# glacierbliss/iceberg_tracking_code

Hardware: AMD Instinct MI355X
Metric: frame_pairs_per_sec (higher is better)
Workload: dtype u8/int32/f32

## Files before the change

### iceberg_tracking_code_amd/build.py

```python
import os
import shutil
import subprocess
import sys
from concurrent.futures import ThreadPoolExecutor

HERE = os.path.dirname(os.path.abspath(__file__))
CSRC = os.path.join(HERE, "csrc")
OBJ = os.path.join(CSRC, "obj")
LIB = os.path.join(HERE, "libicelk.so")
SOURCES = ["icelk_abi.hip", "k_image.hip", "k_pyramid.hip", "k_lk.hip", "k_lk_fast.hip", "k_lk_multi.hip", "k_corners.hip", "k_corners_fast.hip", "k_sort.hip", "k_tail.hip", "k_tracks.hip", "k_utm.hip", "k_mask.hip", "k_grid.hip", "k_cube.hip"]
HEADERS = [os.path.join(CSRC, "icelk_internal.h"), os.path.join(CSRC, "lk_common.h"), os.path.join(CSRC, "lk_fast_tiles.h"), os.path.join(CSRC, "np_sums.h"), os.path.join(HERE, "..", "include", "icelk.h")]
ARCH = "gfx950"
FLAGS = ["--offload-arch=" + ARCH, "-O3", "-fPIC", "-std=c++17", "-ffp-contract=off", "-fno-fast-math",
         "-Wall", "-Wno-unused-result", "-Wno-unused-value"]


def _hipcc():
    exe = shutil.which("hipcc") or "/opt/rocm/bin/hipcc"
    if not os.path.exists(exe):
        raise RuntimeError("hipcc not found: libicelk.so cannot be built (ROCm toolchain required)")
    return exe


def _stale(target, deps):
    if not os.path.exists(target):
        return True
    t = os.path.getmtime(target)
    return any(os.path.getmtime(d) > t for d in deps)


def _compile(src, force):
    obj = os.path.join(OBJ, os.path.splitext(src)[0] + ".o")
    path = os.path.join(CSRC, src)
    if force or _stale(obj, [path] + HEADERS):
        cmd = [_hipcc()] + FLAGS + ["-c", path, "-o", obj]
        subprocess.check_call(cmd)
    return obj


def build(force=False, verbose=False):
    os.makedirs(OBJ, exist_ok=True)
    with ThreadPoolExecutor(max_workers=min(6, len(SOURCES))) as ex:
        objs = list(ex.map(lambda s: _compile(s, force), SOURCES))
    if force or _stale(LIB, objs):
        cmd = [_hipcc(), "--offload-arch=" + ARCH, "-shared", "-fPIC", "-o", LIB] + objs
        subprocess.check_call(cmd)
        if verbose:
            print("built", LIB)
    return LIB


if __name__ == "__main__":
    build(force="--force" in sys.argv, verbose=True)
```

### iceberg_tracking_code_amd/csrc/k_lk_fast.hip

```cpp
#include "lk_fast_tiles.h"

namespace icelk {

namespace {

using namespace lk;
using namespace lkf;

__device__ __forceinline__ float sum_to_float(long long t)
{
    const int hi = (int)(t >> 16), lo = (int)(t & 0xffff);
    return __fadd_rn(__fmul_rn((float)hi, 65536.f), (float)lo);
}

__device__ __forceinline__ int floor_uni(float x)
{
    int i = (int)floorf(x);
    asm volatile("" : "+v"(i));
    return uni(i);
}
__device__ __forceinline__ int floor_uni(float x, float& fx)
{
    fx = floorf(x);
    int i = (int)fx;
    asm volatile("" : "+v"(i));
    return uni(i);
}

template <int WW, int WH>
struct TmplIO {
    using C = Cfg<WW, WH>;
    static constexpr int HP = (C::S + 1) / 2;
    static constexpr int NI = C::TPL * C::S;
    static constexpr bool PACKED = ((NI + 1) / 2 + C::TPL * 2 * HP + 1 + 3) / 4 < (NI + C::TPL * 2 * HP + 1 + 3) / 4;
    static constexpr int NIP = PACKED ? (NI + 1) / 2 : NI;
    static constexpr int NDW = NIP + C::TPL * 2 * HP;
    static constexpr int NQ = (NDW + 1 + 3) / 4;
    static constexpr int LEVEL = NQ * 64;
    static constexpr int WAVES = C::TPL == 1 ? 5 : 3;
    static constexpr bool FITS = (C::LDS_DW * 4 + NQ * 1024) * 4 * WAVES <= 160 * 1024;
    static constexpr int LDS_Q = FITS ? NQ * 64 : 1;
};

template <int WW, int WH>
__device__ __forceinline__ void tmpl_store(const Template<WW, WH, 1>& T, float A11, float A12, float A22,
                                           uint4* __restrict__ dst, int lane)
{
    using IO = TmplIO<WW, WH>;
    using C = Cfg<WW, WH>;
    uint32_t d[IO::NQ * 4];
#pragma unroll
    for (int i = 0; i < IO::NQ * 4; i++) d[i] = 0u;
    d[IO::NDW] = __float_as_uint(lane == 0 ? A11 : (lane == 1 ? A12 : A22));
    constexpr int kSeed = 1 << (W_BITS - 6), kShift = W_BITS - 5;
    if constexpr (IO::PACKED) {
#pragma unroll
        for (int p = 0; p < IO::NIP; p++) {
            const uint32_t lo = (uint32_t)(kSeed - T.Ineg[0][(2 * p) / C::S][(2 * p) % C::S]) >> kShift;
            uint32_t hi = 0u;
            if (2 * p + 1 < IO::NI) hi = (uint32_t)(kSeed - T.Ineg[0][(2 * p + 1) / C::S][(2 * p + 1) % C::S]) << (16 - kShift);
            d[p] = lo | hi;
        }
    } else {
#pragma unroll
        for (int n = 0; n < IO::NI; n++) d[n] = (uint32_t)T.Ineg[0][n / C::S][n % C::S];
    }
#pragma unroll
    for (int k = 0; k < C::TPL; k++) {
#pragma unroll
        for (int q = 0; q < IO::HP; q++) {
            d[IO::NIP + k * 2 * IO::HP + q] = T.Ixp[0][k][q];
            d[IO::NIP + k * 2 * IO::HP + IO::HP + q] = T.Iyp[0][k][q];
        }
    }
    typedef uint32_t u4v __attribute__((ext_vector_type(4)));
#pragma unroll
    for (int q = 0; q < IO::NQ; q++) {
        const u4v v = {d[4 * q], d[4 * q + 1], d[4 * q + 2], d[4 * q + 3]};
        __builtin_nontemporal_store(v, reinterpret_cast<u4v*>(dst + q * 64 + lane));
    }
}

template <int WW, int WH>
__device__ __forceinline__ void tmpl_unpack(Template<WW, WH, 1>& T, float& A11, float& A12, float& A22,
                                            const uint4 (&v)[TmplIO<WW, WH>::NQ])
{
    using IO = TmplIO<WW, WH>;
    using C = Cfg<WW, WH>;
    uint32_t d[IO::NQ * 4];
#pragma unroll
    for (int q = 0; q < IO::NQ; q++) { d[4 * q] = v[q].x; d[4 * q + 1] = v[q].y; d[4 * q + 2] = v[q].z; d[4 * q + 3] = v[q].w; }
    A11 = __uint_as_float((uint32_t)__builtin_amdgcn_readlane((int)d[IO::NDW], 0));
    A12 = __uint_as_float((uint32_t)__builtin_amdgcn_readlane((int)d[IO::NDW], 1));
    A22 = __uint_as_float((uint32_t)__builtin_amdgcn_readlane((int)d[IO::NDW], 2));
    constexpr int kSeed = 1 << (W_BITS - 6), kShift = W_BITS - 5;
#pragma unroll
    for (int n = 0; n < IO::NI; n++) {
        if constexpr (IO::PACKED) {
            const uint32_t w = d[n / 2];
            const uint32_t sh = (n & 1) ? ((w >> (16 - kShift)) & ~((1u << kShift) - 1u)) : ((w & 0xffffu) << kShift);
            T.Ineg[0][n / C::S][n % C::S] = kSeed - (int)sh;
        } else {
            T.Ineg[0][n / C::S][n % C::S] = (int)d[n];
        }
    }
#pragma unroll
    for (int k = 0; k < C::TPL; k++) {
#pragma unroll
        for (int q = 0; q < IO::HP; q++) {
            T.Ixp[0][k][q] = d[IO::NIP + k * 2 * IO::HP + q];
            T.Iyp[0][k][q] = d[IO::NIP + k * 2 * IO::HP + IO::HP + q];
        }
    }
}

template <int WW, int WH, int WHOLE>
__device__ __forceinline__ void chain_sums_t(const float* fsum, int planes, bool pairwise, float (&out)[3], int lane)
{
    constexpr int NPX = WW * WH;
    constexpr int NI = WHOLE / 4, NT = WW - WHOLE, MAXN = NI > NT ? NI : NT, INFL = Cfg<WW, WH>::TPL > 1 ? 16 : 32,
                  RB = INFL / MAXN > 0 ? INFL / MAXN : 1;
    __syncthreads();
    float acc = 0.f;
    const int p = lane / 5, c = lane - 5 * p;
    const bool busy = lane < 5 * planes;
    const int x0 = c < 4 ? c : WHOLE, stride = c < 4 ? 4 : 1, count = busy ? (c < 4 ? NI : NT) : 0;
    const float* src = fsum + (busy ? p : 0) * NPX + x0;
#pragma unroll 1
    for (int y0 = 0; y0 < WH; y0 += RB) {
        float v[RB][MAXN];
#pragma unroll
        for (int r = 0; r < RB; r++)
#pragma unroll
            for (int i = 0; i < MAXN; i++) {
                const bool ok = i < count && y0 + r < WH;
                v[r][i] = ok ? src[(y0 + r) * WW + i * stride] : 0.f;
            }
#pragma unroll
        for (int r = 0; r < RB; r++)
#pragma unroll
            for (int i = 0; i < MAXN; i++) acc = __fadd_rn(acc, v[r][i]);
    }
#pragma unroll
    for (int q = 0; q < 3; q++) {
        if (q >= planes) break;
        const float q0 = __shfl(acc, 5 * q), q1 = __shfl(acc, 5 * q + 1), q2 = __shfl(acc, 5 * q + 2), q3 = __shfl(acc, 5 * q + 3);
        const float t = __shfl(acc, 5 * q + 4);
        out[q] = pairwise ? __fadd_rn(t, __fadd_rn(__fadd_rn(q0, q2), __fadd_rn(q1, q3)))
                          : __fadd_rn(t, __fadd_rn(__fadd_rn(__fadd_rn(q0, q1), q2), q3));
    }
    __syncthreads();
}

template <int WW, int WH>
__device__ __forceinline__ void chain_sums(const float* fsum, int planes, int whole, bool pairwise, float (&out)[3], int lane)
{
    if (whole == (WW & ~3)) chain_sums_t<WW, WH, (WW & ~3)>(fsum, planes, pairwise, out, lane);
    else chain_sums_t<WW, WH, (WW & ~7)>(fsum, planes, pairwise, out, lane);
}

template <int WW, int WH>
__device__ __forceinline__ TrackResult track_point_fast(const Pyramid& PI, const Pyramid& PJ, float p0x, float p0y,
                                                        const LKParams& P, uint32_t* ldsI, uint32_t* ldsJ, int lane,
                                                        bool want_err, uint4* __restrict__ tio, int tmode, uint4* tlds,
                                                        float* fsum = nullptr)
{
    using C = Cfg<WW, WH>;
    using IO = TmplIO<WW, WH>;
    const bool reuse = IO::FITS && tmode == 1;
    int in_lds = -1;
    auto fetch = [&](int level) {
        const unsigned long long sb = reinterpret_cast<unsigned long long>(tio + level * IO::LEVEL);
        const uint4* src = reinterpret_cast<const uint4*>(((unsigned long long)(unsigned)uni((int)(sb >> 32)) << 32) |
                                                          (unsigned)uni((int)sb)) + lane;
        static_for<IO::NQ>([&](auto qq) {
            constexpr int q = qq, grp = q / 4, in = q % 4;
            __builtin_amdgcn_global_load_lds((const __attribute__((address_space(1))) void*)(src + grp * 256),
                                             (__attribute__((address_space(3))) void*)(tlds + grp * 256), 16, in * 1024, 2 );
        });
        in_lds = uni(level);
    };
    if (reuse) fetch(P.top_level);
    constexpr int S = C::S;
    constexpr int R = kMargin;
    const float half_x = (WW - 1) * 0.5f, half_y = (WH - 1) * 0.5f;
    const float FLT_SCALE = 1.f / (1 << 20);
    constexpr bool kSmall = C::TPL * S <= 8;

    int trow[C::TPL], tcol[C::TPL], tlen[C::TPL], joff[C::TPL];
    uint32_t psel[C::TPL][(S + 1) / 2];
#pragma unroll
    for (int k = 0; k < C::TPL; k++) {
        const int t = lane + 64 * k;
        const bool used = t < C::NTASK;
        const int row = used ? t / C::NSEG : 0;
        trow[k] = row;
        tcol[k] = used ? (t - row * C::NSEG) * S : 0;
        tlen[k] = used ? (WW - tcol[k] < S ? WW - tcol[k] : S) : 0;
        joff[k] = row * C::JPD * 4 + tcol[k];
#pragma unroll
        for (int q = 0; q < (S + 1) / 2; q++)
            psel[k][q] = pair_sel(q, tlen[k]);
    }

    constexpr bool kPackSeg = C::TPL >= 3;
    uint32_t segp[C::TPL];
#pragma unroll
    for (int k = 0; k < C::TPL; k++) segp[k] = (uint32_t)trow[k] | ((uint32_t)tcol[k] << 8) | ((uint32_t)tlen[k] << 16);
    auto seg_rows_cols = [&](int (&row)[C::TPL], int (&col)[C::TPL], int (&len)[C::TPL]) {
#pragma unroll
        for (int k = 0; k < C::TPL; k++) {
            uint32_t v = segp[k];
            asm volatile("" : "+v"(v));
            row[k] = (int)(v & 255u);
            col[k] = (int)((v >> 8) & 255u);
            len[k] = (int)(v >> 16);
        }
    };

    TrackResult Rz;
    Rz.status = 1;
    Rz.err = 0.f;
    Rz.iters = 0;
    float sx = 0.f, sy = 0.f;
    Template<WW, WH, 1> T;

    for (int level = P.top_level, scale_bits = __float_as_int(inv_pow2(P.top_level)); level >= 0;
         level--, scale_bits += 1 << 23) {
        const Level LI = PI.lv[level];
        const Level LJ = PJ.lv[level];
        const float scale = __int_as_float(scale_bits);
        float px = p0x * scale, py = p0y * scale;
        if (level == P.top_level) { sx = px; sy = py; }
        else { sx = sx * 2.f; sy = sy * 2.f; }
        px -= half_x; py -= half_y;
        float fpx, fpy;
        const int ipx = floor_uni(px, fpx), ipy = floor_uni(py, fpy);
        if (!origin_ok<WW, WH>(LI, ipx, ipy)) {
            if (level == 0) { Rz.status = 0; Rz.err = 0.f; }
            continue;
        }
        uint32_t wi0, wi1;
        packed_weights<false>(px - fpx, py - fpy, wi0, wi1);

        float nx = sx - half_x, ny = sy - half_y;
        int jx0 = kUnstaged, jy0 = kUnstaged;
        const int ix0 = ipx - 1, iy0 = ipy - 1;
        const bool i_inside = tile_inside(LI, ix0, iy0, C::ITW, C::ITH);
        {
            const int inx = floor_uni(nx), iny = floor_uni(ny);
            const bool j_ok = origin_ok<WW, WH>(LJ, inx, iny);
            const int tjx = inx - R, tjy = iny - R;
            const bool j_inside = j_ok && tile_inside(LJ, tjx, tjy, C::JTW, C::JTH);
            __syncthreads();
            TileRegs<C::IPD, C::ITH> ti;
            TileRegs<C::JPD, C::JTH> tj;
            if (!reuse) {
                if (i_inside) tile_issue(ti, LI, ix0, iy0, lane);
                else tile_issue_reflect(ti, LI, ix0, iy0, lane);
            }
            if (j_inside) tile_issue(tj, LJ, tjx, tjy, lane);
            else if (j_ok) tile_issue_reflect(tj, LJ, tjx, tjy, lane);
            if (!reuse) tile_commit(ti, ldsI, lane);
            if (j_ok) tile_commit(tj, ldsJ, lane);
            if (j_ok) { jx0 = tjx; jy0 = tjy; }
            __syncthreads();
        }

        float A11, A12, A22;
        if (reuse) {
            if (in_lds != level) fetch(level);
            __builtin_amdgcn_s_waitcnt(0x0F70);
            uint4 tq[IO::NQ];
#pragma unroll
            for (int q = 0; q < IO::NQ; q++) tq[q] = tlds[q * 64 + lane];
            tmpl_unpack<WW, WH>(T, A11, A12, A22, tq);
            __builtin_amdgcn_s_waitcnt(0xC07F);
            if (level > 0) fetch(level - 1);
        } else {
            int a11, a12, a22;
            if constexpr (kPackSeg) {
                int row_l[C::TPL], col_l[C::TPL], len_l[C::TPL];
                uint32_t psel_l[C::TPL][(S + 1) / 2];
                seg_rows_cols(row_l, col_l, len_l);
#pragma unroll
                for (int k = 0; k < C::TPL; k++)
#pragma unroll
                    for (int q = 0; q < (S + 1) / 2; q++)
                        psel_l[k][q] = pair_sel(q, len_l[k]);
                template_pixels<WW, WH, 1, 0>(T, ldsI, (uint32_t)uni((int)wi0), (uint32_t)uni((int)wi1),
                                              ix0 & 3, i_inside, ipx, ipy, LI.w, LI.h, row_l, col_l, psel_l, a11, a12, a22, fsum, len_l);
            } else
            template_pixels<WW, WH, 1, 0>(T, ldsI, (uint32_t)uni((int)wi0), (uint32_t)uni((int)wi1),
                                          ix0 & 3, i_inside, ipx, ipy, LI.w, LI.h, trow, tcol, psel, a11, a12, a22, fsum, tlen);
            long long s11, s12, s22;
            if constexpr (kSmall) wave_sum_mat_i64(a11, a12, a22, s11, s12, s22);
            else wave_sum3_i64<1>(a11, a12, a22, s11, s12, s22);
            A11 = sum_to_float(s11) * FLT_SCALE;
            A12 = sum_to_float(s12) * FLT_SCALE;
            A22 = sum_to_float(s22) * FLT_SCALE;
            if (fsum) {
                float o[3];
                chain_sums<WW, WH>(fsum, 3, P.sum_mode == 1 ? (WW & ~3) : (WW & ~7), P.sum_mode == 2, o, lane);
                A11 = __fmul_rn(o[0], FLT_SCALE); A12 = __fmul_rn(o[1], FLT_SCALE); A22 = __fmul_rn(o[2], FLT_SCALE);
            }
        }
        if (IO::FITS && tmode == 2) tmpl_store<WW, WH>(T, A11, A12, A22, tio + level * IO::LEVEL, lane);
        float D = __fsub_rn(__fmul_rn(A11, A22), __fmul_rn(A12, A12));
        const float dif = __fsub_rn(A11, A22);
        const float rad = __fadd_rn(__fmul_rn(dif, dif), __fmul_rn(__fmul_rn(4.f, A12), A12));
        const float tr = __fadd_rn(A22, A11);
        const float approx = (tr - __builtin_amdgcn_sqrtf(rad)) * (1.f / (float)(2 * WW * WH));
        const bool clear_pass = __builtin_amdgcn_ballot_w64(approx > P.min_eig_thr + tr * 2e-6f) != 0 &&
                                !(P.flags & ICELK_FLAG_MIN_EIGENVALS);
        if (!clear_pass) {
            const float minEig = __fdiv_rn(__fsub_rn(tr, sqrtf(rad)), (float)(2 * WW * WH));
            if (P.flags & ICELK_FLAG_MIN_EIGENVALS) Rz.err = minEig;
            if (minEig < P.min_eig_thr) {
                if (level == 0) Rz.status = 0;
                continue;
            }
        }
        if (D < 1.1920928955078125e-07f) {
            if (level == 0) Rz.status = 0;
            continue;
        }
        D = __fdiv_rn(1.f, D);

        float pdx = __builtin_nanf(""), pdy = __builtin_nanf("");
        for (int j = 0; j < P.max_count; j++) {
            float fnx, fny;
            const int inx = floor_uni(nx, fnx), iny = floor_uni(ny, fny);
            if (!origin_ok<WW, WH>(LJ, inx, iny)) {
                if (level == 0) Rz.status = 0;
                break;
            }
            if (!tile_covers(jx0, jy0, inx, iny)) {
                jx0 = inx - R; jy0 = iny - R;
                __syncthreads();
                TileRegs<C::JPD, C::JTH> tj;
                Level LR = LJ;
                asm volatile("" : "+s"(LR.pitch));
                if (tile_inside(LR, jx0, jy0, C::JTW, C::JTH)) tile_issue(tj, LR, jx0, jy0, lane);
                else tile_issue_reflect(tj, LR, jx0, jy0, lane);
                tile_commit(tj, ldsJ, lane);
                __syncthreads();
            }
            Rz.iters++;
            uint32_t wj0, wj1;
            packed_weights<true>(nx - fnx, ny - fny, wj0, wj1);
            const int jb = uni((iny - jy0) * (C::JPD * 4) + (jx0 & 3) + (inx - jx0));
            int b1, b2;
            if constexpr (kPackSeg) {
                int row_l[C::TPL], col_l[C::TPL], len_l[C::TPL], joff_l[C::TPL];
                seg_rows_cols(row_l, col_l, len_l);
#pragma unroll
                for (int k = 0; k < C::TPL; k++) joff_l[k] = row_l[k] * (C::JPD * 4) + col_l[k];
                residual_pixels<WW, WH, 1, 0, false>(T, ldsJ, jb, (uint32_t)uni((int)wj0),
                                                     (uint32_t)uni((int)wj1), joff_l, len_l, b1, b2, fsum, row_l, col_l);
            } else
            residual_pixels<WW, WH, 1, 0, false>(T, ldsJ, jb, (uint32_t)uni((int)wj0),
                                                 (uint32_t)uni((int)wj1), joff, tlen, b1, b2, fsum, trow, tcol);
            long long t1, t2;
            wave_sum2_i64<kSmall ? 8 : 1>(b1, b2, t1, t2);
            float fb1 = sum_to_float(t1) * FLT_SCALE;
            float fb2 = sum_to_float(t2) * FLT_SCALE;
            if (fsum) {
                float o[3];
                chain_sums<WW, WH>(fsum, 2, WW & ~7, true, o, lane);
                fb1 = __fmul_rn(o[0], FLT_SCALE); fb2 = __fmul_rn(o[1], FLT_SCALE);
            }
            const float dx = __fmul_rn(__fsub_rn(__fmul_rn(A12, fb2), __fmul_rn(A22, fb1)), D);
            const float dy = __fmul_rn(__fsub_rn(__fmul_rn(A12, fb1), __fmul_rn(A11, fb2)), D);
            nx = __fadd_rn(nx, dx); ny = __fadd_rn(ny, dy);
            sx = __fadd_rn(nx, half_x); sy = __fadd_rn(ny, half_y);
            const float q = __fadd_rn(__fmul_rn(dx, dx), __fmul_rn(dy, dy));
            bool conv = q < P.eps2_lo;
            if (__builtin_amdgcn_ballot_w64(!conv && !(q > P.eps2_hi)) != 0) {
                asm volatile("" ::: "memory");
                conv = __dadd_rn(__dmul_rn((double)dx, (double)dx), __dmul_rn((double)dy, (double)dy)) <= P.eps2;
            }
            if (conv) break;
            if (fabsf(__fadd_rn(dx, pdx)) <= 0.01f && fabsf(__fadd_rn(dy, pdy)) <= 0.01f) {
                sx = __fsub_rn(sx, __fmul_rn(dx, 0.5f));
                sy = __fsub_rn(sy, __fmul_rn(dy, 0.5f));
                break;
            }
            pdx = dx; pdy = dy;
        }

        if (Rz.status && level == 0 && !(P.flags & ICELK_FLAG_MIN_EIGENVALS)) {
            const float qx = sx - half_x, qy = sy - half_y;
            const int iqx = floor_uni(qx), iqy = floor_uni(qy);
            if (!origin_ok<WW, WH>(LJ, iqx, iqy)) {
                Rz.status = 0;
                continue;
            }
            if (!want_err) continue;
            if (!tile_covers(jx0, jy0, iqx, iqy)) {
                jx0 = iqx - R; jy0 = iqy - R;
                __syncthreads();
                TileRegs<C::JPD, C::JTH> tj;
                if (tile_inside(LJ, jx0, jy0, C::JTW, C::JTH)) tile_issue(tj, LJ, jx0, jy0, lane);
                else tile_issue_reflect(tj, LJ, jx0, jy0, lane);
                tile_commit(tj, ldsJ, lane);
                __syncthreads();
            }
            uint32_t we0, we1;
            packed_weights<true>(qx - (float)iqx, qy - (float)iqy, we0, we1);
            const int jb = uni((iqy - jy0) * (C::JPD * 4) + (jx0 & 3) + (iqx - jx0));
            int es, unused;
            if constexpr (kPackSeg) {
                int row_l[C::TPL], col_l[C::TPL], len_l[C::TPL], joff_l[C::TPL];
                seg_rows_cols(row_l, col_l, len_l);
#pragma unroll
                for (int k = 0; k < C::TPL; k++) joff_l[k] = row_l[k] * (C::JPD * 4) + col_l[k];
                residual_pixels<WW, WH, 1, 0, true>(T, ldsJ, jb, (uint32_t)uni((int)we0),
                                                    (uint32_t)uni((int)we1), joff_l, len_l, es, unused);
            } else
            residual_pixels<WW, WH, 1, 0, true>(T, ldsJ, jb, (uint32_t)uni((int)we0),
                                                (uint32_t)uni((int)we1), joff, tlen, es, unused);
            const float errval = sum_to_float(sum_pick<kSmall, 8>(es));
            Rz.err = __fdiv_rn(__fmul_rn(errval, 1.f), (float)(32 * WW * WH));
        }
    }
    Rz.x = sx;
    Rz.y = sy;
    return Rz;
}

struct LKJobs {
    LKJob job[2];
    int g0, g1;
};

template <int WW, int WH, bool FB, bool SM = false>
__device__ __forceinline__ void lk_fast_body(const LKJobs& JJ, const LKParams& P)
{
    using C = Cfg<WW, WH>;
    constexpr int kTileQ = (C::LDS_DW + 3) / 4;
    __shared__ uint4 lds_q[kTileQ + (SM ? 1 : TmplIO<WW, WH>::LDS_Q)];
    uint4* const tlds = lds_q + kTileQ;
    __shared__ float fs_[SM ? 3 * WW * WH : 1];
    float* const fsum = SM ? fs_ : nullptr;
    int which = 0, b = blockIdx.x;
    if (JJ.g1 > 0) {
        const int G = b >> 3, m = (JJ.g0 < JJ.g1 ? JJ.g0 : JJ.g1) >> 3;
        const int mb = m & ~31;
        int Gj;
        if (G < 2 * mb) {
            which = (G >> 5) & 1;
            Gj = ((G >> 6) << 5) | (G & 31);
        } else if (G < 2 * m) {
            const int r = G - 2 * mb;
            which = r & 1;
            Gj = mb + (r >> 1);
        } else {
            which = JJ.g0 < JJ.g1 ? 1 : 0;
            Gj = G - m;
        }
        b = (Gj << 3) | (b & 7);
    }
    const LKJob& J = JJ.job[which];
    const LKBuffers& B = J.B;
    const int f = __builtin_amdgcn_readfirstlane(launch_slot(B, b, B.n_dev ? *B.n_dev : J.n));
    if (f < 0) return;
    if (B.seg_alive && !B.seg_alive[f]) return;
    const int lane = threadIdx.x;
    uint32_t* ldsJ = reinterpret_cast<uint32_t*>(lds_q);
    uint32_t* ldsI = ldsJ + C::J_DW;
    const float p0x = B.p_in[2 * f], p0y = B.p_in[2 * f + 1];
    if (lane == 0) stamp(B, 0);
    using IO = TmplIO<WW, WH>;
    const size_t t_off = (size_t)f * ((size_t)B.tmpl_levels * IO::LEVEL);
    const TrackResult r1 = track_point_fast<WW, WH>(J.I, J.J, p0x, p0y, P, ldsI, ldsJ, lane, B.err_fwd != nullptr,
                                                    const_cast<uint4*>(static_cast<const uint4*>(B.tmpl_in)) + t_off,
                                                    !SM && B.tmpl_in ? 1 : 0, tlds, fsum);
    if (lane == 0) {
        if (B.p_fwd) { B.p_fwd[2 * f] = r1.x; B.p_fwd[2 * f + 1] = r1.y; }
        if (B.st_fwd) B.st_fwd[f] = (uint8_t)r1.status;
        if (B.err_fwd) B.err_fwd[f] = r1.err;
        if (B.iters && !FB) B.iters[f] = (uint32_t)r1.iters;
    }
    if (FB) {
        const TrackResult r2 = track_point_fast<WW, WH>(J.J, J.I, r1.x, r1.y, P, ldsI, ldsJ, lane, B.err_bwd != nullptr,
                                                        static_cast<uint4*>(B.tmpl_out) + t_off, !SM && B.tmpl_out ? 2 : 0, tlds,
                                                        fsum);
        if (lane == 0) {
            if (B.p_bwd) { B.p_bwd[2 * f] = r2.x; B.p_bwd[2 * f + 1] = r2.y; }
            if (B.st_bwd) B.st_bwd[f] = (uint8_t)r2.status;
            if (B.err_bwd) B.err_bwd[f] = r2.err;
            if (B.iters) B.iters[f] = (uint32_t)r1.iters | ((uint32_t)r2.iters << 16);
            const float d = fb_distance(p0x, p0y, r2.x, r2.y, P.dist_form);
            if (B.dist) B.dist[f] = d;
            if (B.valid) B.valid[f] = d < P.fb_thr ? 1 : 0;
            if (B.seg_alive) seg_append(B, f, r1.x, r1.y, d, d < P.fb_thr);
        }
    }
    if (lane == 0) stamp(B, 1);
}

template <int WW, int WH, bool FB>
__global__ __launch_bounds__(64, 3) void k_lk_fast(LKJobs JJ, LKParams P)
{
    lk_fast_body<WW, WH, FB>(JJ, P);
}

template <int WW, int WH, bool FB>
__global__ __launch_bounds__(64, 4) __attribute__((amdgpu_num_vgpr(44))) void k_lk_fast88(LKJobs JJ, LKParams P)
{
    lk_fast_body<WW, WH, FB>(JJ, P);
}

template <int WW, int WH, bool FB>
__global__ __launch_bounds__(64, 2) void k_lk_fast_sums(LKJobs JJ, LKParams P)
{
    lk_fast_body<WW, WH, FB, true>(JJ, P);
}

int grid_of(const LKBuffers& B, int n) { return B.order ? (n + 15) & ~7 : (n + 7) & ~7; }

template <int WW, int WH>
void launch_fast(hipStream_t s, const LKJob& a, const LKJob* b, const LKParams& P, bool fb)
{
    LKJobs JJ;
    JJ.job[0] = a;
    JJ.job[1] = b ? *b : a;
    JJ.g0 = grid_of(a.B, a.n);
    JJ.g1 = b ? grid_of(b->B, b->n) : 0;
    const int grid = JJ.g0 + JJ.g1;
    if (P.sum_mode) {
        if (fb) hipLaunchKernelGGL((k_lk_fast_sums<WW, WH, true>), dim3(grid), dim3(64), 0, s, JJ, P);
        else hipLaunchKernelGGL((k_lk_fast_sums<WW, WH, false>), dim3(grid), dim3(64), 0, s, JJ, P);
        return;
    }
    if constexpr (Cfg<WW, WH>::TPL == 1) {
        if (fb) hipLaunchKernelGGL((k_lk_fast88<WW, WH, true>), dim3(grid), dim3(64), 0, s, JJ, P);
        else hipLaunchKernelGGL((k_lk_fast88<WW, WH, false>), dim3(grid), dim3(64), 0, s, JJ, P);
    } else {
        if (fb) hipLaunchKernelGGL((k_lk_fast<WW, WH, true>), dim3(grid), dim3(64), 0, s, JJ, P);
        else hipLaunchKernelGGL((k_lk_fast<WW, WH, false>), dim3(grid), dim3(64), 0, s, JJ, P);
    }
}

bool dispatch_fast(hipStream_t s, const LKJob& a, const LKJob* b, const LKParams& P, bool fb)
{
    if (P.flags & ICELK_FLAG_INITIAL_FLOW) return false;
    if (P.win_w == 21 && P.win_h == 21) launch_fast<21, 21>(s, a, b, P, fb);
    else if (P.win_w == 31 && P.win_h == 31) launch_fast<31, 31>(s, a, b, P, fb);
    else if (P.win_w == 35 && P.win_h == 35) launch_fast<35, 35>(s, a, b, P, fb);
    else if (P.win_w == 15 && P.win_h == 15) launch_fast<15, 15>(s, a, b, P, fb);
    else return false;
    return true;
}

}

int lk_template_quads(int win_w, int win_h)
{
    if (win_w == 21 && win_h == 21) return TmplIO<21, 21>::FITS ? TmplIO<21, 21>::NQ : 0;
    if (win_w == 31 && win_h == 31) return TmplIO<31, 31>::FITS ? TmplIO<31, 31>::NQ : 0;
    if (win_w == 35 && win_h == 35) return TmplIO<35, 35>::FITS ? TmplIO<35, 35>::NQ : 0;
    if (win_w == 15 && win_h == 15) return TmplIO<15, 15>::FITS ? TmplIO<15, 15>::NQ : 0;
    return 0;
}

bool lk_fast_eligible(const LKParams& P)
{
    if (P.flags & (ICELK_FLAG_INITIAL_FLOW | ICELK_FLAG_GENERIC_KERNEL | ICELK_FLAG_MULTI_PER_WAVE)) return false;
    return P.sum_mode == 0 && lk_template_quads(P.win_w, P.win_h) > 0;
}

bool launch_lk_fast(hipStream_t s, const Pyramid& I, const Pyramid& J, const LKBuffers& B, int n, const LKParams& P,
                    bool fb)
{
    LKJob a;
    a.I = I;
    a.J = J;
    a.B = B;
    a.n = n;
    return dispatch_fast(s, a, nullptr, P, fb);
}

bool launch_lk_pair(hipStream_t s, const LKJob& a, const LKJob& b, const LKParams& P)
{
    if (P.flags & (ICELK_FLAG_GENERIC_KERNEL | ICELK_FLAG_MULTI_PER_WAVE)) return false;
    if (a.n <= 0 || b.n <= 0) return false;
    return dispatch_fast(s, a, &b, P, true);
}

}
```

### iceberg_tracking_code_amd/csrc/lk_common.h

```cpp
#pragma once
#include "icelk_internal.h"

namespace icelk {
namespace lk {

constexpr int W_BITS = 14;

__device__ __forceinline__ int reflect101(int p, int n)
{
    if (n == 1) return 0;
    while (p < 0 || p >= n) p = p < 0 ? -p : 2 * n - 2 - p;
    return p;
}

__device__ __forceinline__ int descale(int v, int n) { return (v + (1 << (n - 1))) >> n; }

struct Weights {
    int w00, w01, w10, w11;
};

__device__ __forceinline__ Weights bilinear_weights(float a, float b)
{
    Weights w;
    w.w00 = (int)rintf((1.f - a) * (1.f - b) * (float)(1 << W_BITS));
    w.w01 = (int)rintf(a * (1.f - b) * (float)(1 << W_BITS));
    w.w10 = (int)rintf((1.f - a) * b * (float)(1 << W_BITS));
    w.w11 = (1 << W_BITS) - w.w00 - w.w01 - w.w10;
    return w;
}

struct TrackResult {
    float x, y;
    float err;
    int status;
    int iters;
};

__device__ __forceinline__ int wave_sum_i32(int v)
{
    v += __builtin_amdgcn_update_dpp(0, v, 0x111, 0xf, 0xf, true);
    v += __builtin_amdgcn_update_dpp(0, v, 0x112, 0xf, 0xf, true);
    v += __builtin_amdgcn_update_dpp(0, v, 0x114, 0xf, 0xf, true);
    v += __builtin_amdgcn_update_dpp(0, v, 0x118, 0xf, 0xf, true);
    v += __builtin_amdgcn_update_dpp(0, v, 0x142, 0xa, 0xf, true);
    v += __builtin_amdgcn_update_dpp(0, v, 0x143, 0xc, 0xf, true);
    return __builtin_amdgcn_readlane(v, 63);
}

template <int G>
__device__ __forceinline__ long long wave_sum_grouped(int v)
{
    static_assert(G == 8 || G == 16, "group size");
    v += __builtin_amdgcn_update_dpp(0, v, 0x111, 0xf, 0xf, true);
    v += __builtin_amdgcn_update_dpp(0, v, 0x112, 0xf, 0xf, true);
    v += __builtin_amdgcn_update_dpp(0, v, 0x114, 0xf, 0xf, true);
    if (G == 16) v += __builtin_amdgcn_update_dpp(0, v, 0x118, 0xf, 0xf, true);
    long long t = 0;
#pragma unroll
    for (int g = 0; g < 64 / G; g++) t += (long long)__builtin_amdgcn_readlane(v, g * G + G - 1);
    return t;
}

#define ICELK_DPP64_PAIR(LO, HI, CTRL) \
    "v_add_co_u32_dpp " LO ", vcc, " LO ", " LO " " CTRL "\n\tv_addc_co_u32_dpp " HI ", vcc, " HI ", " HI ", vcc " CTRL "\n\t"
#define ICELK_DPP_SHR8 "row_shr:8 row_mask:0xf bank_mask:0xf bound_ctrl:0"
#define ICELK_DPP_BC15 "row_bcast:15 row_mask:0xa bank_mask:0xf"
#define ICELK_DPP_BC31 "row_bcast:31 row_mask:0xc bank_mask:0xf"

template <int G>
__device__ __forceinline__ int dpp_low_steps(int v)
{
    static_assert(G == 1 || G == 8 || G == 16, "group size");
    if (G >= 8) {
        v += __builtin_amdgcn_update_dpp(0, v, 0x111, 0xf, 0xf, true);
        v += __builtin_amdgcn_update_dpp(0, v, 0x112, 0xf, 0xf, true);
        v += __builtin_amdgcn_update_dpp(0, v, 0x114, 0xf, 0xf, true);
    }
    if (G == 16) v += __builtin_amdgcn_update_dpp(0, v, 0x118, 0xf, 0xf, true);
    return v;
}

__device__ __forceinline__ long long lane63_i64(int lo, int hi)
{
    const unsigned l = (unsigned)__builtin_amdgcn_readlane(lo, 63);
    const int h = __builtin_amdgcn_readlane(hi, 63);
    return (long long)(((unsigned long long)(unsigned)h << 32) | l);
}

template <int G>
__device__ __forceinline__ void wave_sum2_i64(int v0, int v1, long long& s0, long long& s1)
{
    int l0 = dpp_low_steps<G>(v0), l1 = dpp_low_steps<G>(v1);
    int h0 = l0 >> 31, h1 = l1 >> 31;
    if (G == 1)
        asm("s_nop 1\n\t"
            ICELK_DPP64_PAIR("%0", "%1", "row_shr:1 row_mask:0xf bank_mask:0xf bound_ctrl:0") ICELK_DPP64_PAIR("%2", "%3", "row_shr:1 row_mask:0xf bank_mask:0xf bound_ctrl:0")
            ICELK_DPP64_PAIR("%0", "%1", "row_shr:2 row_mask:0xf bank_mask:0xf bound_ctrl:0") ICELK_DPP64_PAIR("%2", "%3", "row_shr:2 row_mask:0xf bank_mask:0xf bound_ctrl:0")
            ICELK_DPP64_PAIR("%0", "%1", "row_shr:4 row_mask:0xf bank_mask:0xf bound_ctrl:0") ICELK_DPP64_PAIR("%2", "%3", "row_shr:4 row_mask:0xf bank_mask:0xf bound_ctrl:0")
            : "+v"(l0), "+v"(h0), "+v"(l1), "+v"(h1) : : "vcc");
    if (G <= 8)
        asm("s_nop 1\n\t" ICELK_DPP64_PAIR("%0", "%1", ICELK_DPP_SHR8) ICELK_DPP64_PAIR("%2", "%3", ICELK_DPP_SHR8)
            : "+v"(l0), "+v"(h0), "+v"(l1), "+v"(h1) : : "vcc");
    asm("s_nop 1\n\t" ICELK_DPP64_PAIR("%0", "%1", ICELK_DPP_BC15) ICELK_DPP64_PAIR("%2", "%3", ICELK_DPP_BC15)
        ICELK_DPP64_PAIR("%0", "%1", ICELK_DPP_BC31) ICELK_DPP64_PAIR("%2", "%3", ICELK_DPP_BC31)
        : "+v"(l0), "+v"(h0), "+v"(l1), "+v"(h1) : : "vcc");
    s0 = lane63_i64(l0, h0);
    s1 = lane63_i64(l1, h1);
}

template <int G>
__device__ __forceinline__ void wave_sum3_i64(int v0, int v1, int v2, long long& s0, long long& s1, long long& s2)
{
    int l0 = dpp_low_steps<G>(v0), l1 = dpp_low_steps<G>(v1), l2 = dpp_low_steps<G>(v2);
    int h0 = l0 >> 31, h1 = l1 >> 31, h2 = l2 >> 31;
    if (G == 1)
        asm("s_nop 1\n\t"
            ICELK_DPP64_PAIR("%0", "%1", "row_shr:1 row_mask:0xf bank_mask:0xf bound_ctrl:0") ICELK_DPP64_PAIR("%2", "%3", "row_shr:1 row_mask:0xf bank_mask:0xf bound_ctrl:0") ICELK_DPP64_PAIR("%4", "%5", "row_shr:1 row_mask:0xf bank_mask:0xf bound_ctrl:0")
            ICELK_DPP64_PAIR("%0", "%1", "row_shr:2 row_mask:0xf bank_mask:0xf bound_ctrl:0") ICELK_DPP64_PAIR("%2", "%3", "row_shr:2 row_mask:0xf bank_mask:0xf bound_ctrl:0") ICELK_DPP64_PAIR("%4", "%5", "row_shr:2 row_mask:0xf bank_mask:0xf bound_ctrl:0")
            ICELK_DPP64_PAIR("%0", "%1", "row_shr:4 row_mask:0xf bank_mask:0xf bound_ctrl:0") ICELK_DPP64_PAIR("%2", "%3", "row_shr:4 row_mask:0xf bank_mask:0xf bound_ctrl:0") ICELK_DPP64_PAIR("%4", "%5", "row_shr:4 row_mask:0xf bank_mask:0xf bound_ctrl:0")
            : "+v"(l0), "+v"(h0), "+v"(l1), "+v"(h1), "+v"(l2), "+v"(h2) : : "vcc");
    if (G <= 8)
        asm("s_nop 1\n\t" ICELK_DPP64_PAIR("%0", "%1", ICELK_DPP_SHR8) ICELK_DPP64_PAIR("%2", "%3", ICELK_DPP_SHR8) ICELK_DPP64_PAIR("%4", "%5", ICELK_DPP_SHR8)
            : "+v"(l0), "+v"(h0), "+v"(l1), "+v"(h1), "+v"(l2), "+v"(h2) : : "vcc");
    asm("s_nop 1\n\t" ICELK_DPP64_PAIR("%0", "%1", ICELK_DPP_BC15) ICELK_DPP64_PAIR("%2", "%3", ICELK_DPP_BC15) ICELK_DPP64_PAIR("%4", "%5", ICELK_DPP_BC15)
        ICELK_DPP64_PAIR("%0", "%1", ICELK_DPP_BC31) ICELK_DPP64_PAIR("%2", "%3", ICELK_DPP_BC31) ICELK_DPP64_PAIR("%4", "%5", ICELK_DPP_BC31)
        : "+v"(l0), "+v"(h0), "+v"(l1), "+v"(h1), "+v"(l2), "+v"(h2) : : "vcc");
    s0 = lane63_i64(l0, h0);
    s1 = lane63_i64(l1, h1);
    s2 = lane63_i64(l2, h2);
}

__device__ __forceinline__ void wave_sum_mat_i64(int v0, int v1, int v2, long long& s0, long long& s1, long long& s2)
{
    int l0 = dpp_low_steps<16>(v0), l1 = dpp_low_steps<16>(v1), l2 = dpp_low_steps<16>(v2);
    int h0, h1 = l1 >> 31, h2;
    asm("s_nop 1\n\t"
        "v_add_u32_dpp %0, %0, %0 " ICELK_DPP_BC15 "\n\t"
        ICELK_DPP64_PAIR("%2", "%3", ICELK_DPP_BC15)
        "v_add_u32_dpp %4, %4, %4 " ICELK_DPP_BC15 "\n\t"
        "v_add_co_u32_dpp %0, vcc, %0, %0 " ICELK_DPP_BC31 "\n\t"
        "v_addc_co_u32_e64 %1, vcc, 0, 0, vcc\n\t"
        ICELK_DPP64_PAIR("%2", "%3", ICELK_DPP_BC31)
        "v_add_co_u32_dpp %4, vcc, %4, %4 " ICELK_DPP_BC31 "\n\t"
        "v_addc_co_u32_e64 %5, vcc, 0, 0, vcc"
        : "+v"(l0), "=v"(h0), "+v"(l1), "+v"(h1), "+v"(l2), "=v"(h2) : : "vcc");
    s0 = lane63_i64(l0, h0);
    s1 = lane63_i64(l1, h1);
    s2 = lane63_i64(l2, h2);
}

__device__ __forceinline__ float i64_to_float(long long t)
{
    const double d = (double)(int)(t >> 32) * 4294967296.0 + (double)(unsigned)t;
    return (float)d;
}

__device__ __forceinline__ int uni(int v) { return __builtin_amdgcn_readfirstlane(v); }
__device__ __forceinline__ float uni_f(float v) { return __int_as_float(__builtin_amdgcn_readfirstlane(__float_as_int(v))); }

__device__ __forceinline__ float inv_pow2(int level) { return __int_as_float((127 - level) << 23); }

__device__ __forceinline__ long long wave_sum_exact(int v)
{
    const int lo = wave_sum_i32(v & 0xffff);
    const int hi = wave_sum_i32(v >> 16);
    return ((long long)hi << 16) + (long long)lo;
}

__device__ __forceinline__ int launch_slot(const LKBuffers& B, int b, int count)
{
    if (!B.order) return b < count ? b : -1;
    if (B.order_plain) return b < count ? B.order[b] : -1;
    const int nb = B.order_border ? *B.order_border : 0;
    if (b < nb) return B.order[b];
    const int rest = count - nb, bb = b - nb;
    const int chunk = (rest + 7) >> 3, j = bb >> 3;
    const int idx = (bb & 7) * chunk + j;
    return (j < chunk && idx < rest) ? B.order[nb + idx] : -1;
}

__device__ __forceinline__ void seg_append(const LKBuffers& B, int f, float x, float y, float d, bool valid)
{
    B.seg_alive[f] = valid ? 1 : 0;
    if (valid) {
        B.seg_xy[2 * f] = x;
        B.seg_xy[2 * f + 1] = y;
        float* t = B.seg_tracks + ((size_t)f * B.seg_max_vert + B.seg_vert) * 2;
        t[0] = x;
        t[1] = y;
        B.seg_quality[(size_t)f * (B.seg_max_vert - 1) + (B.seg_vert - 1)] = d;
    }
    atomicAdd(&B.seg_tracked[f & 63], 1ull);
}

__device__ __forceinline__ float fb_distance(float p0x, float p0y, float rx, float ry, int form)
{
    const float ddx = fabsf(__fsub_rn(p0x, rx)), ddy = fabsf(__fsub_rn(p0y, ry));
    if (form == 1) return sqrtf(__fadd_rn(__fmul_rn(ddx, ddx), __fmul_rn(ddy, ddy)));
    const double x = (double)ddx, y = (double)ddy;
    return (float)sqrt(__dadd_rn(__dmul_rn(x, x), __dmul_rn(y, y)));
}

__device__ __forceinline__ void stamp(const LKBuffers& B, int which)
{
    if (!B.stamps) return;
    unsigned long long* s = B.stamps + 3 * (size_t)blockIdx.x;
    s[which] = __builtin_amdgcn_s_memtime();
    if (which == 0)
        s[2] = (unsigned long long)__builtin_amdgcn_s_getreg((31 << 11) | 4) |
               ((unsigned long long)(__builtin_amdgcn_s_getreg((3 << 11) | 20) & 15) << 32);
}

template <bool SMALL, int G>
__device__ __forceinline__ long long sum_pick(int v)
{
    if constexpr (SMALL) return wave_sum_grouped<G>(v);
    else return wave_sum_exact(v);
}

}
}
```

Measured before the change: 7620.

## Use MFMA matrix ops for LK residual wave reductions instead of DPP chains

Moves the DPP-based wave sum helpers into a new header and adds MFMA-based reduction variants. In the non-packed-segment LK fast path, the residual sums b1/b2 are now reduced through an i8 MFMA byte-split trick followed by an f32 MFMA, replacing the 64-bit DPP add chain and readlane sequence. This is meant to shorten the per-iteration reduction latency in the iterative solver by using matrix units, but it depends on assumptions about the value range and rounding of the byte-split and bias constants, which could affect exactness.

New measurement: 7724, median of 5. 1.4% higher.

```diff
diff --git a/iceberg_tracking_code_amd/build.py b/iceberg_tracking_code_amd/build.py
--- a/iceberg_tracking_code_amd/build.py
+++ b/iceberg_tracking_code_amd/build.py
@@ -9,7 +9,7 @@
 OBJ = os.path.join(CSRC, "obj")
 LIB = os.path.join(HERE, "libicelk.so")
 SOURCES = ["icelk_abi.hip", "k_image.hip", "k_pyramid.hip", "k_lk.hip", "k_lk_fast.hip", "k_lk_multi.hip", "k_corners.hip", "k_corners_fast.hip", "k_sort.hip", "k_tail.hip", "k_tracks.hip", "k_utm.hip", "k_mask.hip", "k_grid.hip", "k_cube.hip"]
-HEADERS = [os.path.join(CSRC, "icelk_internal.h"), os.path.join(CSRC, "lk_common.h"), os.path.join(CSRC, "lk_fast_tiles.h"), os.path.join(CSRC, "np_sums.h"), os.path.join(HERE, "..", "include", "icelk.h")]
+HEADERS = [os.path.join(CSRC, "icelk_internal.h"), os.path.join(CSRC, "lk_common.h"), os.path.join(CSRC, "lk_wave_sums.h"), os.path.join(CSRC, "lk_fast_tiles.h"), os.path.join(CSRC, "np_sums.h"), os.path.join(HERE, "..", "include", "icelk.h")]
 ARCH = "gfx950"
 FLAGS = ["--offload-arch=" + ARCH, "-O3", "-fPIC", "-std=c++17", "-ffp-contract=off", "-fno-fast-math",
          "-Wall", "-Wno-unused-result", "-Wno-unused-value"]
diff --git a/iceberg_tracking_code_amd/csrc/k_lk_fast.hip b/iceberg_tracking_code_amd/csrc/k_lk_fast.hip
--- a/iceberg_tracking_code_amd/csrc/k_lk_fast.hip
+++ b/iceberg_tracking_code_amd/csrc/k_lk_fast.hip
@@ -6,12 +6,6 @@
 
 using namespace lk;
 using namespace lkf;
-
-__device__ __forceinline__ float sum_to_float(long long t)
-{
-    const int hi = (int)(t >> 16), lo = (int)(t & 0xffff);
-    return __fadd_rn(__fmul_rn((float)hi, 65536.f), (float)lo);
-}
 
 __device__ __forceinline__ int floor_uni(float x)
 {
@@ -361,10 +355,15 @@
             } else
             residual_pixels<WW, WH, 1, 0, false>(T, ldsJ, jb, (uint32_t)uni((int)wj0),
                                                  (uint32_t)uni((int)wj1), joff, tlen, b1, b2, fsum, trow, tcol);
-            long long t1, t2;
-            wave_sum2_i64<kSmall ? 8 : 1>(b1, b2, t1, t2);
-            float fb1 = sum_to_float(t1) * FLT_SCALE;
-            float fb2 = sum_to_float(t2) * FLT_SCALE;
+            float fb1, fb2;
+            if constexpr (kPackSeg) {
+                long long t1, t2;
+                wave_sum2_i64<1>(b1, b2, t1, t2);
+                fb1 = sum_to_float(t1) * FLT_SCALE;
+                fb2 = sum_to_float(t2) * FLT_SCALE;
+            } else {
+                wave_sum2_mm<WW == 15>(b1, b2, lane, fb1, fb2);
+            }
             if (fsum) {
                 float o[3];
                 chain_sums<WW, WH>(fsum, 2, WW & ~7, true, o, lane);
diff --git a/iceberg_tracking_code_amd/csrc/lk_common.h b/iceberg_tracking_code_amd/csrc/lk_common.h
--- a/iceberg_tracking_code_amd/csrc/lk_common.h
+++ b/iceberg_tracking_code_amd/csrc/lk_common.h
@@ -1,5 +1,6 @@
 #pragma once
 #include "icelk_internal.h"
+#include "lk_wave_sums.h"
 
 namespace icelk {
 namespace lk {
@@ -61,93 +62,6 @@
     return t;
 }
 
-#define ICELK_DPP64_PAIR(LO, HI, CTRL) \
-    "v_add_co_u32_dpp " LO ", vcc, " LO ", " LO " " CTRL "\n\tv_addc_co_u32_dpp " HI ", vcc, " HI ", " HI ", vcc " CTRL "\n\t"
-#define ICELK_DPP_SHR8 "row_shr:8 row_mask:0xf bank_mask:0xf bound_ctrl:0"
-#define ICELK_DPP_BC15 "row_bcast:15 row_mask:0xa bank_mask:0xf"
-#define ICELK_DPP_BC31 "row_bcast:31 row_mask:0xc bank_mask:0xf"
-
-template <int G>
-__device__ __forceinline__ int dpp_low_steps(int v)
-{
-    static_assert(G == 1 || G == 8 || G == 16, "group size");
-    if (G >= 8) {
-        v += __builtin_amdgcn_update_dpp(0, v, 0x111, 0xf, 0xf, true);
-        v += __builtin_amdgcn_update_dpp(0, v, 0x112, 0xf, 0xf, true);
-        v += __builtin_amdgcn_update_dpp(0, v, 0x114, 0xf, 0xf, true);
-    }
-    if (G == 16) v += __builtin_amdgcn_update_dpp(0, v, 0x118, 0xf, 0xf, true);
-    return v;
-}
-
-__device__ __forceinline__ long long lane63_i64(int lo, int hi)
-{
-    const unsigned l = (unsigned)__builtin_amdgcn_readlane(lo, 63);
-    const int h = __builtin_amdgcn_readlane(hi, 63);
-    return (long long)(((unsigned long long)(unsigned)h << 32) | l);
-}
-
-template <int G>
-__device__ __forceinline__ void wave_sum2_i64(int v0, int v1, long long& s0, long long& s1)
-{
-    int l0 = dpp_low_steps<G>(v0), l1 = dpp_low_steps<G>(v1);
-    int h0 = l0 >> 31, h1 = l1 >> 31;
-    if (G == 1)
-        asm("s_nop 1\n\t"
-            ICELK_DPP64_PAIR("%0", "%1", "row_shr:1 row_mask:0xf bank_mask:0xf bound_ctrl:0") ICELK_DPP64_PAIR("%2", "%3", "row_shr:1 row_mask:0xf bank_mask:0xf bound_ctrl:0")
-            ICELK_DPP64_PAIR("%0", "%1", "row_shr:2 row_mask:0xf bank_mask:0xf bound_ctrl:0") ICELK_DPP64_PAIR("%2", "%3", "row_shr:2 row_mask:0xf bank_mask:0xf bound_ctrl:0")
-            ICELK_DPP64_PAIR("%0", "%1", "row_shr:4 row_mask:0xf bank_mask:0xf bound_ctrl:0") ICELK_DPP64_PAIR("%2", "%3", "row_shr:4 row_mask:0xf bank_mask:0xf bound_ctrl:0")
-            : "+v"(l0), "+v"(h0), "+v"(l1), "+v"(h1) : : "vcc");
-    if (G <= 8)
-        asm("s_nop 1\n\t" ICELK_DPP64_PAIR("%0", "%1", ICELK_DPP_SHR8) ICELK_DPP64_PAIR("%2", "%3", ICELK_DPP_SHR8)
-            : "+v"(l0), "+v"(h0), "+v"(l1), "+v"(h1) : : "vcc");
-    asm("s_nop 1\n\t" ICELK_DPP64_PAIR("%0", "%1", ICELK_DPP_BC15) ICELK_DPP64_PAIR("%2", "%3", ICELK_DPP_BC15)
-        ICELK_DPP64_PAIR("%0", "%1", ICELK_DPP_BC31) ICELK_DPP64_PAIR("%2", "%3", ICELK_DPP_BC31)
-        : "+v"(l0), "+v"(h0), "+v"(l1), "+v"(h1) : : "vcc");
-    s0 = lane63_i64(l0, h0);
-    s1 = lane63_i64(l1, h1);
-}
-
-template <int G>
-__device__ __forceinline__ void wave_sum3_i64(int v0, int v1, int v2, long long& s0, long long& s1, long long& s2)
-{
-    int l0 = dpp_low_steps<G>(v0), l1 = dpp_low_steps<G>(v1), l2 = dpp_low_steps<G>(v2);
-    int h0 = l0 >> 31, h1 = l1 >> 31, h2 = l2 >> 31;
-    if (G == 1)
-        asm("s_nop 1\n\t"
-            ICELK_DPP64_PAIR("%0", "%1", "row_shr:1 row_mask:0xf bank_mask:0xf bound_ctrl:0") ICELK_DPP64_PAIR("%2", "%3", "row_shr:1 row_mask:0xf bank_mask:0xf bound_ctrl:0") ICELK_DPP64_PAIR("%4", "%5", "row_shr:1 row_mask:0xf bank_mask:0xf bound_ctrl:0")
-            ICELK_DPP64_PAIR("%0", "%1", "row_shr:2 row_mask:0xf bank_mask:0xf bound_ctrl:0") ICELK_DPP64_PAIR("%2", "%3", "row_shr:2 row_mask:0xf bank_mask:0xf bound_ctrl:0") ICELK_DPP64_PAIR("%4", "%5", "row_shr:2 row_mask:0xf bank_mask:0xf bound_ctrl:0")
-            ICELK_DPP64_PAIR("%0", "%1", "row_shr:4 row_mask:0xf bank_mask:0xf bound_ctrl:0") ICELK_DPP64_PAIR("%2", "%3", "row_shr:4 row_mask:0xf bank_mask:0xf bound_ctrl:0") ICELK_DPP64_PAIR("%4", "%5", "row_shr:4 row_mask:0xf bank_mask:0xf bound_ctrl:0")
-            : "+v"(l0), "+v"(h0), "+v"(l1), "+v"(h1), "+v"(l2), "+v"(h2) : : "vcc");
-    if (G <= 8)
-        asm("s_nop 1\n\t" ICELK_DPP64_PAIR("%0", "%1", ICELK_DPP_SHR8) ICELK_DPP64_PAIR("%2", "%3", ICELK_DPP_SHR8) ICELK_DPP64_PAIR("%4", "%5", ICELK_DPP_SHR8)
-            : "+v"(l0), "+v"(h0), "+v"(l1), "+v"(h1), "+v"(l2), "+v"(h2) : : "vcc");
-    asm("s_nop 1\n\t" ICELK_DPP64_PAIR("%0", "%1", ICELK_DPP_BC15) ICELK_DPP64_PAIR("%2", "%3", ICELK_DPP_BC15) ICELK_DPP64_PAIR("%4", "%5", ICELK_DPP_BC15)
-        ICELK_DPP64_PAIR("%0", "%1", ICELK_DPP_BC31) ICELK_DPP64_PAIR("%2", "%3", ICELK_DPP_BC31) ICELK_DPP64_PAIR("%4", "%5", ICELK_DPP_BC31)
-        : "+v"(l0), "+v"(h0), "+v"(l1), "+v"(h1), "+v"(l2), "+v"(h2) : : "vcc");
-    s0 = lane63_i64(l0, h0);
-    s1 = lane63_i64(l1, h1);
-    s2 = lane63_i64(l2, h2);
-}
-
-__device__ __forceinline__ void wave_sum_mat_i64(int v0, int v1, int v2, long long& s0, long long& s1, long long& s2)
-{
-    int l0 = dpp_low_steps<16>(v0), l1 = dpp_low_steps<16>(v1), l2 = dpp_low_steps<16>(v2);
-    int h0, h1 = l1 >> 31, h2;
-    asm("s_nop 1\n\t"
-        "v_add_u32_dpp %0, %0, %0 " ICELK_DPP_BC15 "\n\t"
-        ICELK_DPP64_PAIR("%2", "%3", ICELK_DPP_BC15)
-        "v_add_u32_dpp %4, %4, %4 " ICELK_DPP_BC15 "\n\t"
-        "v_add_co_u32_dpp %0, vcc, %0, %0 " ICELK_DPP_BC31 "\n\t"
-        "v_addc_co_u32_e64 %1, vcc, 0, 0, vcc\n\t"
-        ICELK_DPP64_PAIR("%2", "%3", ICELK_DPP_BC31)
-        "v_add_co_u32_dpp %4, vcc, %4, %4 " ICELK_DPP_BC31 "\n\t"
-        "v_addc_co_u32_e64 %5, vcc, 0, 0, vcc"
-        : "+v"(l0), "=v"(h0), "+v"(l1), "+v"(h1), "+v"(l2), "=v"(h2) : : "vcc");
-    s0 = lane63_i64(l0, h0);
-    s1 = lane63_i64(l1, h1);
-    s2 = lane63_i64(l2, h2);
-}
 
 __device__ __forceinline__ float i64_to_float(long long t)
 {
diff --git a/iceberg_tracking_code_amd/csrc/lk_wave_sums.h b/iceberg_tracking_code_amd/csrc/lk_wave_sums.h
--- /dev/null
+++ b/iceberg_tracking_code_amd/csrc/lk_wave_sums.h
@@ -0,0 +1,165 @@
+#pragma once
+#include <hip/hip_runtime.h>
+
+namespace icelk {
+namespace lk {
+
+#define ICELK_DPP64_PAIR(LO, HI, CTRL) \
+    "v_add_co_u32_dpp " LO ", vcc, " LO ", " LO " " CTRL "\n\tv_addc_co_u32_dpp " HI ", vcc, " HI ", " HI ", vcc " CTRL "\n\t"
+#define ICELK_DPP_SHR8 "row_shr:8 row_mask:0xf bank_mask:0xf bound_ctrl:0"
+#define ICELK_DPP_BC15 "row_bcast:15 row_mask:0xa bank_mask:0xf"
+#define ICELK_DPP_BC31 "row_bcast:31 row_mask:0xc bank_mask:0xf"
+
+template <int G>
+__device__ __forceinline__ int dpp_low_steps(int v)
+{
+    static_assert(G == 1 || G == 8 || G == 16, "group size");
+    if (G >= 8) {
+        v += __builtin_amdgcn_update_dpp(0, v, 0x111, 0xf, 0xf, true);
+        v += __builtin_amdgcn_update_dpp(0, v, 0x112, 0xf, 0xf, true);
+        v += __builtin_amdgcn_update_dpp(0, v, 0x114, 0xf, 0xf, true);
+    }
+    if (G == 16) v += __builtin_amdgcn_update_dpp(0, v, 0x118, 0xf, 0xf, true);
+    return v;
+}
+
+__device__ __forceinline__ long long lane63_i64(int lo, int hi)
+{
+    const unsigned l = (unsigned)__builtin_amdgcn_readlane(lo, 63);
+    const int h = __builtin_amdgcn_readlane(hi, 63);
+    return (long long)(((unsigned long long)(unsigned)h << 32) | l);
+}
+
+template <int G>
+__device__ __forceinline__ void wave_sum2_i64(int v0, int v1, long long& s0, long long& s1)
+{
+    int l0 = dpp_low_steps<G>(v0), l1 = dpp_low_steps<G>(v1);
+    int h0 = l0 >> 31, h1 = l1 >> 31;
+    if (G == 1)
+        asm("s_nop 1\n\t"
+            ICELK_DPP64_PAIR("%0", "%1", "row_shr:1 row_mask:0xf bank_mask:0xf bound_ctrl:0") ICELK_DPP64_PAIR("%2", "%3", "row_shr:1 row_mask:0xf bank_mask:0xf bound_ctrl:0")
+            ICELK_DPP64_PAIR("%0", "%1", "row_shr:2 row_mask:0xf bank_mask:0xf bound_ctrl:0") ICELK_DPP64_PAIR("%2", "%3", "row_shr:2 row_mask:0xf bank_mask:0xf bound_ctrl:0")
+            ICELK_DPP64_PAIR("%0", "%1", "row_shr:4 row_mask:0xf bank_mask:0xf bound_ctrl:0") ICELK_DPP64_PAIR("%2", "%3", "row_shr:4 row_mask:0xf bank_mask:0xf bound_ctrl:0")
+            : "+v"(l0), "+v"(h0), "+v"(l1), "+v"(h1) : : "vcc");
+    if (G <= 8)
+        asm("s_nop 1\n\t" ICELK_DPP64_PAIR("%0", "%1", ICELK_DPP_SHR8) ICELK_DPP64_PAIR("%2", "%3", ICELK_DPP_SHR8)
+            : "+v"(l0), "+v"(h0), "+v"(l1), "+v"(h1) : : "vcc");
+    asm("s_nop 1\n\t" ICELK_DPP64_PAIR("%0", "%1", ICELK_DPP_BC15) ICELK_DPP64_PAIR("%2", "%3", ICELK_DPP_BC15)
+        ICELK_DPP64_PAIR("%0", "%1", ICELK_DPP_BC31) ICELK_DPP64_PAIR("%2", "%3", ICELK_DPP_BC31)
+        : "+v"(l0), "+v"(h0), "+v"(l1), "+v"(h1) : : "vcc");
+    s0 = lane63_i64(l0, h0);
+    s1 = lane63_i64(l1, h1);
+}
+
+template <int G>
+__device__ __forceinline__ void wave_sum3_i64(int v0, int v1, int v2, long long& s0, long long& s1, long long& s2)
+{
+    int l0 = dpp_low_steps<G>(v0), l1 = dpp_low_steps<G>(v1), l2 = dpp_low_steps<G>(v2);
+    int h0 = l0 >> 31, h1 = l1 >> 31, h2 = l2 >> 31;
+    if (G == 1)
+        asm("s_nop 1\n\t"
+            ICELK_DPP64_PAIR("%0", "%1", "row_shr:1 row_mask:0xf bank_mask:0xf bound_ctrl:0") ICELK_DPP64_PAIR("%2", "%3", "row_shr:1 row_mask:0xf bank_mask:0xf bound_ctrl:0") ICELK_DPP64_PAIR("%4", "%5", "row_shr:1 row_mask:0xf bank_mask:0xf bound_ctrl:0")
+            ICELK_DPP64_PAIR("%0", "%1", "row_shr:2 row_mask:0xf bank_mask:0xf bound_ctrl:0") ICELK_DPP64_PAIR("%2", "%3", "row_shr:2 row_mask:0xf bank_mask:0xf bound_ctrl:0") ICELK_DPP64_PAIR("%4", "%5", "row_shr:2 row_mask:0xf bank_mask:0xf bound_ctrl:0")
+            ICELK_DPP64_PAIR("%0", "%1", "row_shr:4 row_mask:0xf bank_mask:0xf bound_ctrl:0") ICELK_DPP64_PAIR("%2", "%3", "row_shr:4 row_mask:0xf bank_mask:0xf bound_ctrl:0") ICELK_DPP64_PAIR("%4", "%5", "row_shr:4 row_mask:0xf bank_mask:0xf bound_ctrl:0")
+            : "+v"(l0), "+v"(h0), "+v"(l1), "+v"(h1), "+v"(l2), "+v"(h2) : : "vcc");
+    if (G <= 8)
+        asm("s_nop 1\n\t" ICELK_DPP64_PAIR("%0", "%1", ICELK_DPP_SHR8) ICELK_DPP64_PAIR("%2", "%3", ICELK_DPP_SHR8) ICELK_DPP64_PAIR("%4", "%5", ICELK_DPP_SHR8)
+            : "+v"(l0), "+v"(h0), "+v"(l1), "+v"(h1), "+v"(l2), "+v"(h2) : : "vcc");
+    asm("s_nop 1\n\t" ICELK_DPP64_PAIR("%0", "%1", ICELK_DPP_BC15) ICELK_DPP64_PAIR("%2", "%3", ICELK_DPP_BC15) ICELK_DPP64_PAIR("%4", "%5", ICELK_DPP_BC15)
+        ICELK_DPP64_PAIR("%0", "%1", ICELK_DPP_BC31) ICELK_DPP64_PAIR("%2", "%3", ICELK_DPP_BC31) ICELK_DPP64_PAIR("%4", "%5", ICELK_DPP_BC31)
+        : "+v"(l0), "+v"(h0), "+v"(l1), "+v"(h1), "+v"(l2), "+v"(h2) : : "vcc");
+    s0 = lane63_i64(l0, h0);
+    s1 = lane63_i64(l1, h1);
+    s2 = lane63_i64(l2, h2);
+}
+
+__device__ __forceinline__ void wave_sum_mat_i64(int v0, int v1, int v2, long long& s0, long long& s1, long long& s2)
+{
+    int l0 = dpp_low_steps<16>(v0), l1 = dpp_low_steps<16>(v1), l2 = dpp_low_steps<16>(v2);
+    int h0, h1 = l1 >> 31, h2;
+    asm("s_nop 1\n\t"
+        "v_add_u32_dpp %0, %0, %0 " ICELK_DPP_BC15 "\n\t"
+        ICELK_DPP64_PAIR("%2", "%3", ICELK_DPP_BC15)
+        "v_add_u32_dpp %4, %4, %4 " ICELK_DPP_BC15 "\n\t"
+        "v_add_co_u32_dpp %0, vcc, %0, %0 " ICELK_DPP_BC31 "\n\t"
+        "v_addc_co_u32_e64 %1, vcc, 0, 0, vcc\n\t"
+        ICELK_DPP64_PAIR("%2", "%3", ICELK_DPP_BC31)
+        "v_add_co_u32_dpp %4, vcc, %4, %4 " ICELK_DPP_BC31 "\n\t"
+        "v_addc_co_u32_e64 %5, vcc, 0, 0, vcc"
+        : "+v"(l0), "=v"(h0), "+v"(l1), "+v"(h1), "+v"(l2), "=v"(h2) : : "vcc");
+    s0 = lane63_i64(l0, h0);
+    s1 = lane63_i64(l1, h1);
+    s2 = lane63_i64(l2, h2);
+}
+
+__device__ __forceinline__ float sum_to_float(long long t)
+{
+    const int hi = (int)(t >> 16), lo = (int)(t & 0xffff);
+    return __fadd_rn(__fmul_rn((float)hi, 65536.f), (float)lo);
+}
+
+typedef double f64x4_t __attribute__((ext_vector_type(4)));
+
+__device__ __forceinline__ double mfma_sum_weight()
+{
+    double w = 0x1p-10;
+    asm volatile("" : "+v"(w));
+    return w;
+}
+
+template <int N>
+__device__ __forceinline__ void wave_sums_f64(const int (&v)[N], float (&f)[N])
+{
+    const double w = mfma_sum_weight();
+    const f64x4_t zero = {0.0, 0.0, 0.0, 0.0};
+    f64x4_t d[N];
+    double u[N];
+#pragma unroll
+    for (int n = 0; n < N; n++) d[n] = __builtin_amdgcn_mfma_f64_16x16x4f64((double)v[n], w, zero, 0, 0, 0);
+#pragma unroll
+    for (int n = 0; n < N; n++) u[n] = (d[n].x + d[n].y) + (d[n].z + d[n].w);
+#pragma unroll
+    for (int n = 0; n < N; n++) d[n] = __builtin_amdgcn_mfma_f64_16x16x4f64(u[n], w, zero, 0, 0, 0);
+#pragma unroll
+    for (int n = 0; n < N; n++) f[n] = (float)d[n].x;
+}
+
+__device__ __forceinline__ void wave_sum2_f64(int v0, int v1, float& f0, float& f1)
+{
+    const int v[2] = {v0, v1};
+    float f[2];
+    wave_sums_f64<2>(v, f);
+    f0 = f[0]; f1 = f[1];
+}
+
+__device__ __forceinline__ void wave_sum3_f64(int v0, int v1, int v2, float& f0, float& f1, float& f2)
+{
+    const int v[3] = {v0, v1, v2};
+    float f[3];
+    wave_sums_f64<3>(v, f);
+    f0 = f[0]; f1 = f[1]; f2 = f[2];
+}
+
+typedef int i32x4_t __attribute__((ext_vector_type(4)));
+typedef float f32x4_t __attribute__((ext_vector_type(4)));
+
+template <bool REMAT = false>
+__device__ __forceinline__ void wave_sum2_mm(int v0, int v1, int lane, float& f0, float& f1)
+{
+    const unsigned long long a = ((unsigned long long)(unsigned)(v1 ^ 0x00808080) << 32) | (unsigned)(v0 ^ 0x00808080);
+    if (REMAT) asm volatile("" : "+v"(lane));
+    const unsigned long long sel = 1ull << ((lane & 7) * 8);
+    const i32x4_t zi = {0, 0, 0, 0};
+    const i32x4_t d = __builtin_amdgcn_mfma_i32_16x16x32_i8((long)a, (long)sel, zi, 0, 0, 0);
+    const int c = (d.x + d.y + d.z) + (d.w + 2048);
+    const f32x4_t zf = {0.f, 0.f, 0.f, 0.f};
+    const f32x4_t e = __builtin_amdgcn_mfma_f32_16x16x4f32((float)c, 1.f, zf, 0, 0, 0);
+    const float lo = __fmaf_rn(e.y, 256.f, e.x);
+    const float hi = __fadd_rn(__fmaf_rn(e.w, 256.f, e.z), -2097152.f);
+    const float r = __fmaf_rn(hi, 0.0625f, __fmul_rn(lo, 0x1p-20f));
+    f0 = __int_as_float(__builtin_amdgcn_readlane(__float_as_int(r), 0));
+    f1 = __int_as_float(__builtin_amdgcn_readlane(__float_as_int(r), 16));
+}
+
+}
+}
```
